# CoolMicApp/libcoolmic-dsp

Hardware: AMD Instinct MI355X
Metric: Msamples/s transform->vumeter (higher is better)
Workload: dtype int16

## Files before the change

### libcoolmic-dsp_amd/__init__.py

```python
import ctypes as C
import os

import numpy as np

_HERE = os.path.dirname(os.path.abspath(__file__))
LIB_PATH = os.environ.get("COOLMIC_HIP_LIB") or os.path.join(_HERE, "lib", "libcoolmic-dsp-hip.so")
if not os.path.exists(LIB_PATH):
    raise ImportError(
        f"{LIB_PATH} is missing: build it with `make -C {_HERE}` "
        "(or __graft_entry__.build()); there is no CPU fallback")

lib = C.CDLL(LIB_PATH)

MAX_CH = 16
ssize_t = C.c_ssize_t

ERROR_NONE, ERROR_GENERIC, ERROR_NOSYS, ERROR_FAULT = 0, -1, -8, -9
ERROR_INVAL, ERROR_NOMEM, ERROR_BUSY = -10, -11, -12

OUT_PCM, OUT_F32, VU, INPLACE, EQ, HOSTPCM, EXTSLOTS = 0x1, 0x2, 0x4, 0x8, 0x10, 0x20, 0x40
PLACE_SEARCH = 0x80
GEN_NULL, GEN_SINE, GEN_NOISE = 0, 1, 2
VU_FINISH_HOST, VU_FINISH_DEVICE = 0, 1
NODE_WORDS = 34
# ... 214 lines not shown
    "coolmic_group_get_iohandle": (_vp, [_vp, C.c_uint]),
    "coolmic_group_pump": (C.c_int, [_vp]),
    "coolmic_group_set_pull_threads": (C.c_int, [_vp, C.c_uint]),
    "coolmic_group_vumeter_result": (C.c_int, [_vp, C.c_uint, _P(VuResult)]),
    "coolmic_group_vumeter_results": (C.c_int, [_vp, _vp, _vp]),
    "coolmic_group_set_vu_finish": (C.c_int, [_vp, C.c_int]),
    "coolmic_group_set_true_peak": (C.c_int, [_vp, C.c_int]),
    "coolmic_group_true_peak": (C.c_int, [_vp, C.c_uint, _P(TruePeakResult)]),
    "coolmic_group_true_peaks": (C.c_int, [_vp, _vp, _vp]),
    "coolmic_group_set_loudness": (C.c_int, [_vp, C.c_int]),
    "coolmic_group_loudness": (C.c_int, [_vp, C.c_uint, _P(LoudnessResult)]),
    "coolmic_group_loudnesses": (C.c_int, [_vp, _vp, _vp]),
    "coolmic_group_loudness_set_weights": (C.c_int, [_vp, C.c_long, _vp]),
    "coolmic_group_loudness_reset": (C.c_int, [_vp, C.c_long]),
    "coolmic_group_streams": (C.c_uint, [_vp]),
}
MISSING = []
for _name, (_res, _args) in SIGNATURES.items():
    if not hasattr(lib, _name):
        MISSING.append(_name)
        continue
    _fn = getattr(lib, _name)
    _fn.restype = _res
    if _args is not None:
        _fn.argtypes = _args

if hasattr(lib, "cmhip_test_gain_consts"):
    lib.cmhip_test_gain_consts.restype = None
    lib.cmhip_test_gain_consts.argtypes = [C.c_uint16, C.c_uint16, _P(C.c_uint16), _P(C.c_uint32)]
if hasattr(lib, "cmhip_test_plan_run"):
    lib.cmhip_test_plan_run.restype = None
    lib.cmhip_test_plan_run.argtypes = [C.c_uint32, C.c_uint32, C.c_uint32, C.c_int, C.c_int, C.c_int, C.c_int,
                                        C.c_void_p]
lib.cmhip_test_merge_windows.restype = C.c_int
lib.cmhip_test_merge_windows.argtypes = [_P(C.c_uint64), C.c_uint, C.c_uint, C.c_uint, _P(VuResult)]
if hasattr(lib, "cmhip_test_unpack_finished"):
    lib.cmhip_test_unpack_finished.restype = C.c_int
    lib.cmhip_test_unpack_finished.argtypes = [_vp, C.c_uint, C.c_uint, C.c_uint, _vp, _vp]
    lib.cmhip_test_power_db_device.restype = C.c_int
    lib.cmhip_test_power_db_device.argtypes = [_vp, _vp, C.c_uint, _vp, _vp]
if hasattr(lib, "cmhip_test_plan_tpeak"):
    lib.cmhip_test_plan_tpeak.restype = None
    lib.cmhip_test_plan_tpeak.argtypes = [C.c_uint32, C.c_uint32, C.c_uint32, C.c_void_p]
    lib.cmhip_debug_tp_count.restype = C.c_ulonglong
    lib.cmhip_debug_tp_count.argtypes = []
if hasattr(lib, "cmhip_test_plan_loud"):
    lib.cmhip_test_plan_loud.restype = None
    lib.cmhip_test_plan_loud.argtypes = [C.c_uint32, C.c_uint32, C.c_uint32, C.c_void_p]
    lib.cmhip_debug_loud_count.restype = C.c_ulonglong
    lib.cmhip_debug_loud_count.argtypes = []
if hasattr(lib, "cmhip_test_plan_src"):
    lib.cmhip_test_plan_src.restype = None
    lib.cmhip_test_plan_src.argtypes = [C.c_uint32] * 6 + [C.c_void_p]
lib.cmhip_debug_run_count.restype = C.c_ulonglong
lib.cmhip_debug_run_count.argtypes = []
lib.coolmic_debug_vumeter_mode.restype = C.c_int
lib.coolmic_debug_vumeter_mode.argtypes = [_vp]
lib.coolmic_sine_period.restype = C.c_int
lib.coolmic_sine_period.argtypes = [C.c_uint32, _vp, _P(C.c_size_t)]


class CoolmicError(RuntimeError):
    def __init__(self, what, code):
        text = lib.coolmic_error2string(code).decode()
        detail = lib.cmhip_last_error().decode()
        super().__init__(f"{what}: {code} ({text}) {detail}")
# ... 2 lines not shown

def _check(what, rc):
    if rc != ERROR_NONE:
        raise CoolmicError(what, rc)


def device_count():
    return lib.cmhip_device_count()


def device_synchronize(device=0):
    _check("device_synchronize", lib.cmhip_device_synchronize(device))


def device_mem_info(device=0):
    f, t = C.c_size_t(), C.c_size_t()
    _check("device_mem_info", lib.cmhip_device_mem_info(device, C.byref(f), C.byref(t)))
    return f.value, t.value


def last_error():
    return lib.cmhip_last_error().decode()


def gain_consts(gain, scale):
    mi, mf = C.c_uint16(), C.c_uint32()
    lib.cmhip_test_gain_consts(gain, scale, C.byref(mi), C.byref(mf))
    return mi.value, mf.value


class RunPlan(C.Structure):
    _fields_ = [(name, C.c_int if name == "err" else C.c_uint32)
                for name in ("err", "family", "channels", "tile_u", "waves", "map", "stage", "grid", "block",
                             "chunks", "W", "rows_per_tile", "keep_flag")]


class TpPlan(C.Structure):
    _fields_ = [("err", C.c_int), ("fast", C.c_uint32), ("grid", C.c_uint32), ("block", C.c_uint32),
                ("chunks", C.c_uint32)]


def plan_tpeak(streams, channels, frames):
    p = TpPlan()
    lib.cmhip_test_plan_tpeak(streams, channels, frames, C.addressof(p))
    return p


def tp_dbtp(peak):
    return lib.cmhip_tp_dbtp(peak)


def tp_coefficients():
    h = np.zeros(48, dtype=np.int16)
    lib.cmhip_tp_coefficients(h.ctypes.data)
    return h.reshape(4, 12)


class LoudPlan(C.Structure):
    _fields_ = [("err", C.c_int), ("vec", C.c_uint32), ("grid", C.c_uint32), ("block", C.c_uint32)]


def plan_loud(streams, channels, frames):
    p = LoudPlan()
    lib.cmhip_test_plan_loud(streams, channels, frames, C.addressof(p))
    return p


# ... 17 lines not shown
class SrcPlan(C.Structure):
    _fields_ = [("err", C.c_int)] + [(n, C.c_uint32) for n in ("fast", "grid", "block", "chunks", "tile_out", "tile_in",
                                                               "row", "table_lds", "lds_bytes")]


def plan_src(streams, channels, L, M, T, out_frames):
    p = SrcPlan()
    lib.cmhip_test_plan_src(streams, channels, L, M, T, out_frames, C.addressof(p))
    return p


def src_design(rate_in, rate_out):
    L, M, T = C.c_uint(), C.c_uint(), C.c_uint()
    _check("src_design", lib.cmhip_src_design(rate_in, rate_out, C.byref(L), C.byref(M), C.byref(T), None, 0))
    h = np.zeros(L.value * T.value, dtype=np.int16)
    _check("src_design", lib.cmhip_src_design(rate_in, rate_out, None, None, None, h.ctypes.data, h.size))
    return L.value, M.value, T.value, h.reshape(L.value, T.value)


def src_out_frames(L, M, r, frames):
    return lib.cmhip_src_out_frames(L, M, r, frames)


RUN_FAMILIES = ("none", "fast", "fast_ro", "wide", "rows")


def plan_run(streams, channels, frames, out=False, f32=False, vu=False, identity_maps=True):
    p = RunPlan()
    lib.cmhip_test_plan_run(streams, channels, frames, int(bool(out)), int(bool(f32)), int(bool(vu)),
                            int(bool(identity_maps)), C.byref(p))
    d = {name: getattr(p, name) for name, _ in RunPlan._fields_}
    d["family"] = RUN_FAMILIES[d["family"]]
    return d


def merge_windows(windows, channels, rate=48000):
    import numpy as np
    w = np.ascontiguousarray(windows, dtype=np.uint64).reshape(-1, 33)
    r = VuResult()
    rc = lib.cmhip_test_merge_windows(w.ctypes.data_as(_P(C.c_uint64)), w.shape[0], channels, rate, C.byref(r))
    return rc, r


def unpack_finished(words, streams, channels, rate=48000, out=None):
    w = np.ascontiguousarray(words, dtype=np.uint64).reshape(-1)
    out = out if out is not None else (VuResult * streams)()
    rc = (C.c_int * streams)()
    _check("unpack_finished", lib.cmhip_test_unpack_finished(w.ctypes.data, streams, channels, rate, out, rc))
    return out, list(rc)


def power_db_device(sums, counts, want_log=False):
    s = np.ascontiguousarray(sums, dtype=np.uint64)
    c = np.ascontiguousarray(counts, dtype=np.uint64)
    assert s.shape == c.shape and s.ndim == 1
    db = np.empty(s.size, dtype=np.float64)
    lg = np.empty(s.size, dtype=np.float64) if want_log else None
    _check("power_db_device", lib.cmhip_test_power_db_device(s.ctypes.data, c.ctypes.data, s.size, db.ctypes.data,
                                                             lg.ctypes.data if want_log else None))
    return (db, lg) if want_log else db


def sine_period(rate):
    buf = np.zeros(96, dtype=np.int16)
    n = C.c_size_t()
    rc = lib.coolmic_sine_period(rate, buf.ctypes.data, C.byref(n))
# ... 728 lines not shown
```

### libcoolmic-dsp_amd/csrc/cmhip_device.h

```cpp
#ifndef CMHIP_DEVICE_H
#define CMHIP_DEVICE_H

#include "cmhip_internal.h"
#include <stdlib.h>
#include <type_traits>

namespace cmhip {

using u32 = uint32_t;
using u64 = unsigned long long;
typedef unsigned int u32x4 __attribute__((ext_vector_type(4)));
typedef unsigned int u32x2 __attribute__((ext_vector_type(2)));
typedef float f32x4 __attribute__((ext_vector_type(4)));


__device__ __forceinline__ u32 uniform(u32 v) { return __builtin_amdgcn_readfirstlane(v); }

__device__ __forceinline__ void done_epilogue(uint32_t *flag, uint32_t seq)
{
    if (flag) {
        __threadfence_system();
        __syncthreads();
        if (threadIdx.x == 0)
            __hip_atomic_store(flag, seq, __ATOMIC_RELEASE, __HIP_MEMORY_SCOPE_SYSTEM);
    }
}

__device__ __forceinline__ u64 make_key(u32 mag, u64 index, u32 neg)
{
    if (mag == 0)
        return 0;
    return ((u64)mag << KEY_ABS_SHIFT) | ((~index & KEY_IDX_MASK) << 1) | (u64)neg;
}


typedef short v2s __attribute__((ext_vector_type(2)));
typedef unsigned short v2u __attribute__((ext_vector_type(2)));

__device__ __forceinline__ u32 pk_sign(u32 w)
{
    v2s v = __builtin_bit_cast(v2s, w);
    v = v >> (short)15;
    return __builtin_bit_cast(u32, v);
}
__device__ __forceinline__ u32 pk_sub(u32 a, u32 b)
{
    v2u x = __builtin_bit_cast(v2u, a) - __builtin_bit_cast(v2u, b);
    return __builtin_bit_cast(u32, x);
}
// ... 59 lines not shown
__device__ __forceinline__ void with_gain_mode(u32 mode, F &&f)
{
    if constexpr (MODES) {
        if (mode == GAIN_IDENTITY)
            f(std::integral_constant<u32, GAIN_IDENTITY>{});
        else if (mode == GAIN_BELOW_SCALE)
            f(std::integral_constant<u32, GAIN_BELOW_SCALE>{});
        else
            f(std::integral_constant<u32, GAIN_GENERAL>{});
    } else {
        f(std::integral_constant<u32, GAIN_GENERAL>{});
    }
}

template <u32 N>
__device__ __forceinline__ int half_at(const u32 (&o)[N], u32 j)
{
    u32 w = 0;
#pragma unroll
    for (u32 i = 0; i < N; i++)
        if (i == (j >> 1))
            w = o[i];
    return (int)(short)(w >> (16u * (j & 1u)));
}

struct Extent {
    u32 nfr, nsamp;
    u32 nfull;
    u32 ntail;
};
__device__ __forceinline__ Extent stream_extent(const uint32_t *nframes, u32 frames, u32 s, u32 C)
{
    Extent e;
    e.nfr = nframes ? nframes[s] : frames;
    e.nsamp = e.nfr * C;
    e.nfull = e.nsamp >> 3;
    e.ntail = e.nsamp & 7u;
    return e;
}

__device__ __forceinline__ void load_vec(u32 (&x)[4], const int16_t *ins, u32 v, bool full, bool tail, u32 ntail)
{
    u32x4 w = {0, 0, 0, 0};
    if (full)
        w = __builtin_nontemporal_load(reinterpret_cast<const u32x4 *>(ins) + v);
    x[0] = w.x; x[1] = w.y; x[2] = w.z; x[3] = w.w;
    if (tail) {
        for (u32 j = 0; j < ntail; j++) {
            const u32 val = (u32)(uint16_t)ins[(u64)v * 8 + j];
#pragma unroll
            for (u32 i = 0; i < 4; i++)
                if (i == (j >> 1))
                    x[i] |= val << (16u * (j & 1u));
        }
    }
}
__device__ __forceinline__ void store_tail(int16_t *outs, u32 v, const u32 (&o)[4], u32 ntail)
{
    for (u32 j = 0; j < ntail; j++)
        outs[(u64)v * 8 + j] = (int16_t)half_at(o, j);
}

__device__ __forceinline__ u64 window_base(const RunArgs &a, VuState *vs, u32 k, u32 nsamp)
{
    const u64 base = vs->samples[a.parity];
    if (k == 0 && (threadIdx.x & 63u) == 0)
        vs->samples[a.parity ^ 1u] = base + nsamp;
    return base;
}

struct PeakAt {
    u32 u, lane, first, neg;
};
template <u32 NS, u32 TU>
__device__ __forceinline__ PeakAt locate_peak(u32 wkey, const u32 (&qw)[TU][4], const u32 (&x)[TU][4], u32 slot)
{
    const u32 mag = wkey >> 16;
    PeakAt p = {TU - 1u - ((wkey >> 6) & (TU - 1u)), 63u - (wkey & 63u), 8, 0};
    u32 Q[4], X[4];
#pragma unroll
    for (u32 u = 0; u < TU; u++) {
        if (p.u == u) {
#pragma unroll
            for (u32 i = 0; i < 4; i++) {
                Q[i] = (u32)__builtin_amdgcn_readlane((int)qw[u][i], (int)p.lane);
                X[i] = (u32)__builtin_amdgcn_readlane((int)x[u][i], (int)p.lane);
            }
        }
    }
#pragma unroll
    for (u32 j = 0; j < 8; j++) {
        if (j % NS != slot)
            continue;
        if (((u32)half_at(Q, j) & 0xffffu) == mag && p.first == 8) {
            p.first = j;
            p.neg = half_at(X, j) < 0 ? 1u : 0u;
        }
    }
    return p;
}

// ... 128 lines not shown
```

### libcoolmic-dsp_amd/csrc/cmhip_internal.h

```cpp
#pragma once

#include <hip/hip_runtime.h>
#include <hip/hip_ext.h>
#include <stdint.h>

namespace cmhip {

constexpr unsigned MAX_CH = 16;
constexpr unsigned MAX_EQ = 4;

struct alignas(128) StreamParam {
    uint32_t mode;
    uint32_t perm2;
    uint32_t map_identity;
    uint32_t mi01;
    uint32_t mf[MAX_CH];
    uint16_t mi[MAX_CH];
    uint8_t  chmap[MAX_CH];
};
static_assert(sizeof(StreamParam) == 128, "one line per stream");
constexpr uint32_t GAIN_GENERAL = 0, GAIN_BELOW_SCALE = 1, GAIN_IDENTITY = 2;

struct VuState {
    unsigned long long power[MAX_CH];
    unsigned long long key[MAX_CH];
    unsigned long long samples[2];
};

constexpr int      KEY_ABS_SHIFT = 47;
constexpr uint64_t KEY_IDX_MASK  = (1ull << 46) - 1;
constexpr int      NODE_KEY_ABS_SHIFT = 46;

struct EqParam {
    uint32_t nsec;
    float    coef[MAX_EQ][5];
};
struct EqState {
    float s[MAX_EQ][4];
};

struct RunArgs {
    const int16_t *in;
    int16_t       *out;
    float         *f32;
    const StreamParam *param;
    VuState       *vu;
    const uint32_t *nframes;
    uint32_t       frames;
    uint32_t       streams;
    uint32_t       channels;
    uint64_t       stride;
    uint64_t       plane;
    uint32_t       chunks;
    uint32_t       parity;
    uint32_t       identity_maps;
    uint32_t      *done_flag;
    uint32_t       done_seq;
};

struct EqArgs {
    const int16_t *in;
    int16_t       *out;
    float         *f32;
    const StreamParam *param;
    const EqParam *eq;
    EqState       *state;
    VuState       *vu;
    const uint32_t *nframes;
    uint32_t       frames;
    uint32_t       streams;
    uint32_t       channels;
    uint32_t       nsec;
    uint32_t       whole_streams;
    uint32_t       parity;
    uint64_t       stride;
    uint64_t       plane;
    uint32_t      *done_flag;
    uint32_t       done_seq;
};

constexpr unsigned TP_TAPS = 12;
constexpr unsigned TP_HIST = TP_TAPS - 1;
constexpr int16_t TP_P0[TP_TAPS] = {14, 90, -161, 272, -487, 1125, 7964, -838, 390, -218, 122, -68};
constexpr int16_t TP_P1[TP_TAPS] = {-239, 240, -424, 730, -1364, 3810, 6388, -1641, 832, -477, 271, -155};
constexpr int16_t tp_h(unsigned p, unsigned k)
{
    return p == 0 ? TP_P0[k] : p == 1 ? TP_P1[k] : p == 2 ? TP_P1[TP_TAPS - 1 - k] : TP_P0[TP_TAPS - 1 - k];
}

struct TpArgs {
// ... 47 lines not shown
    uint32_t       frames;
    uint32_t       streams;
    uint32_t       channels;
    uint32_t       parity;
    uint32_t       L, M, T;
    uint32_t       inv_l;
    uint32_t       chunks;
    uint32_t       tile_out;
    uint32_t       row;
    uint32_t       table_lds;
};

struct GenArgs {
    int16_t *dst;
    uint32_t streams, channels, frames;
    uint64_t stride;
    uint32_t seed;
    uint64_t first_global, global_step, frame_offset;
    int16_t  sine[48];
};

enum RunFamily : uint32_t { RUN_NONE = 0, RUN_FAST, RUN_FAST_RO, RUN_WIDE, RUN_ROWS };
struct RunPlan {
    hipError_t err;
    uint32_t   family;
    uint32_t   channels;
    uint32_t   tile_u;
    uint32_t   waves;
    uint32_t   map, stage;
    uint32_t   grid, block;
    uint32_t   chunks;
    uint32_t   W, rows_per_tile;
    uint32_t   keep_flag;
};
RunPlan plan_run(const RunArgs &a);
hipError_t launch_run(const RunArgs &a, hipStream_t st, hipEvent_t ev_start = nullptr, hipEvent_t ev_stop = nullptr,
                      bool *flagged = nullptr);
hipError_t prepare_eq(int device);
hipError_t launch_eq(const EqArgs &a, hipStream_t st, hipEvent_t ev_start = nullptr, hipEvent_t ev_stop = nullptr,
                     bool *flagged = nullptr);
struct TpPlan {
    hipError_t err;
    uint32_t   fast;
    uint32_t   grid, block;
    uint32_t   chunks;
};
TpPlan plan_tpeak(const TpArgs &a);
hipError_t launch_tpeak(const TpArgs &a, hipStream_t st);
struct LoudPlan {
    hipError_t err;
    uint32_t   vec;
    uint32_t   grid, block;
};
LoudPlan plan_loud(const LoudArgs &a);
hipError_t launch_loud(const LoudArgs &a, hipStream_t st);
struct SrcPlan {
    hipError_t err;
    uint32_t   fast;
    uint32_t   grid, block;
    uint32_t   chunks;
    uint32_t   tile_out;
    uint32_t   tile_in;
    uint32_t   row;
    uint32_t   table_lds;
    uint32_t   lds_bytes;
};
// ... 18 lines not shown
```

### libcoolmic-dsp_amd/csrc/k_block.hip

```cpp
#include "cmhip_device.h"

namespace cmhip {

constexpr u32 TILE_U_VUONLY = 16;

struct FastShare {
    u64 sum[2], key[2];
    u32 arrived;
};

template <int C, bool WRITE_PCM, bool WRITE_F32, bool DO_VU, int U, bool FULL>
__device__ __forceinline__ void fast_tile(const RunArgs &a, u32 s, u32 k, u32 nsamp, u32 nfull, u32 ntail,
                                          u64 base, VuState *vs, FastShare *share, const int16_t *a_in,
                                          int16_t *a_out, u64 a_stride)
{
    constexpr u32 TILE_U = U;
    constexpr u32 TILE_VEC = 64 * TILE_U;
    const u32 lane = threadIdx.x & 63u;
    const u32 v0 = k * TILE_VEC;

    const int16_t *ins = a_in + (u64)s * a_stride;
    int16_t *outs = WRITE_PCM ? a_out + (u64)s * a_stride : nullptr;
    u32x4 *dst = reinterpret_cast<u32x4 *>(outs);
    float *f32s = WRITE_F32 ? a.f32 + (u64)s * a.plane * C : nullptr;

    u32 x[TILE_U][4];
    bool full[TILE_U], tail[TILE_U];
#pragma unroll
    for (u32 u = 0; u < TILE_U; u++) {
        const u32 v = v0 + 64u * u + lane;
        full[u] = FULL || v < nfull;
        tail[u] = !FULL && ntail && v == nfull;
        load_vec(x[u], ins, v, full[u], tail[u], ntail);
    }

    __builtin_amdgcn_sched_barrier(0);
    (void)nsamp;
    const StreamParam *p = a.param + s;
    const u32 perm2 = p->perm2;
    constexpr bool ROLES = C == 2 && DO_VU && !WRITE_PCM && !WRITE_F32;
    const bool keep = ROLES && (perm2 == 0x03020100u || perm2 == 0x01000302u);
    const u32 sw = keep && perm2 == 0x01000302u ? 1u : 0u;
    const u32 mi01 = p->mi01;
    const u32 mf0 = p->mf[0], mf1 = p->mf[C - 1];
    const u32 mipk = C == 1 ? (mi01 & 0xffffu) * 0x10001u : (sw ? (mi01 >> 16) | (mi01 << 16) : mi01);
    const u32 mflo = sw ? mf1 : mf0, mfhi = sw ? mf0 : mf1;
    constexpr bool MODES = DO_VU && !WRITE_PCM && FULL;
    const u32 mode = MODES ? uniform(p->mode) : GAIN_GENERAL;

    if constexpr (ROLES) {
        if (!keep) {
#pragma unroll
            for (u32 u = 0; u < TILE_U; u++)
#pragma unroll
                for (u32 i = 0; i < 4; i++)
                    x[u][i] = __builtin_amdgcn_perm(x[u][i], x[u][i], perm2);
        }
    }

    u32 qw[TILE_U][4];
    PowAcc pw[2] = {{0, 0, 0}, {0, 0, 0}};
    u32 best[2] = {0, 0};
    __shared__ __attribute__((aligned(16))) float fst[WRITE_F32 && C == 1 && FULL ? 64 * 8 : 4];
    auto arithmetic = [&](auto mode_c) {
    constexpr u32 MODE = decltype(mode_c)::value;
#pragma unroll
    for (u32 u = 0; u < TILE_U; u++) {
        const u32 v = v0 + 64u * u + lane;
        u32 o[4], vmax = 0;
#pragma unroll
        for (u32 i = 0; i < 4; i++) {
// ... 44 lines not shown
            } else if constexpr (WRITE_F32) {
                store_f32<C>(f32s, a.plane, v, o);
            }
        } else if (tail[u]) {
            for (u32 j = 0; j < ntail; j++) {
                const int q = half_at(o, j);
                if constexpr (WRITE_PCM)
                    outs[(u64)v * 8 + j] = (int16_t)q;
                if constexpr (WRITE_F32)
                    f32s[(u64)(j % (u32)C) * a.plane + ((u64)v * 8 + j) / (u32)C] = q * (1.0f / 32768.0f);
            }
        }
    }
    };
    with_gain_mode<MODES>(mode, arithmetic);

    if constexpr (DO_VU) {
        pw[0].flush();
        pw[1].flush();
        u64 sum[2];
        u32 wkey[2];
        if constexpr (C == 1) {
            sum[0] = wave_add_u40(pw[0].total + pw[1].total);
            wkey[0] = wave_max_u32(max(best[0], best[1]));
            sum[1] = 0;
            wkey[1] = 0;
        } else {
            sum[0] = wave_add_u40(pw[0].total);
            sum[1] = wave_add_u40(pw[1].total);
            wkey[0] = wave_max_u32(best[0]);
            wkey[1] = wave_max_u32(best[1]);
        }
        u64 gkey[2] = {0, 0};
#pragma unroll
        for (int c = 0; c < C; c++) {
            const u32 mag = wkey[c] >> 16;
            if (mag == 0)
                continue;
            const PeakAt pk = locate_peak<(u32)C>(wkey[c], qw, x, (u32)c);
            gkey[c] = make_key(mag, base + 8ull * (v0 + 64u * pk.u + pk.lane) + (pk.first ^ sw), pk.neg);
        }
        if (lane < (u32)C) {
            const u64 ssum = (lane ^ sw) == 0 ? sum[0] : sum[1];
            const u64 skey = (lane ^ sw) == 0 ? gkey[0] : gkey[1];
            if (share) {
                if (ssum)
                    atomicAdd(&share->sum[lane], ssum);
                if (skey)
                    atomicMax(&share->key[lane], skey);
            } else {
                if (ssum)
                    atomicAdd(&vs->power[lane], ssum);
                if (skey)
                    atomicMax(&vs->key[lane], skey);
            }
        }
    }
}

template <int C, bool WRITE_PCM, bool WRITE_F32, bool DO_VU, int U, int NW = 1>
__device__ __forceinline__ void run_fast(const RunArgs &a)
{
    constexpr u32 TILE_VEC = 64 * U;
    static_assert(NW == 1 || !WRITE_F32, "the float-plane forms stage through LDS with one-wave barriers");
    const u32 lane = threadIdx.x & 63u;
    const int16_t *a_in = a.in;
    int16_t *a_out = a.out;
    const u64 a_stride = a.stride;
    const u32 a_frames = a.frames;
    u32 s, k;
    if constexpr (NW == 1) {
        s = blockIdx.x / a.chunks;
        k = blockIdx.x - s * a.chunks;
    } else {
        const u32 cw = (a.chunks + (u32)NW - 1u) / (u32)NW;
        s = blockIdx.x / cw;
        k = (blockIdx.x - s * cw) * (u32)NW + (threadIdx.x >> 6);
    }
    __shared__ FastShare shared_;
    FastShare *share = NW > 1 && DO_VU ? &shared_ : nullptr;
    if constexpr (NW > 1 && DO_VU) {
        if (threadIdx.x < 2u) {
            shared_.sum[threadIdx.x] = 0;
            shared_.key[threadIdx.x] = 0;
        }
        if (threadIdx.x == 0)
            shared_.arrived = 0;
        __syncthreads();
    }

    const Extent e = stream_extent(a.nframes, a_frames, s, (u32)C);
    const u32 nsamp = e.nsamp, nfull = e.nfull, ntail = e.ntail;
    const u32 v0 = k * TILE_VEC;

    VuState *vs = DO_VU ? a.vu + s : nullptr;
    u64 base = 0;
    if constexpr (DO_VU)
        base = window_base(a, vs, k, nsamp);
    if (v0 >= nfull + (ntail ? 1u : 0u)) {
        if constexpr (NW == 1)
            return;
    } else if (v0 + TILE_VEC <= nfull) {
        fast_tile<C, WRITE_PCM, WRITE_F32, DO_VU, U, true>(a, s, k, nsamp, nfull, ntail, base, vs, share, a_in, a_out, a_stride);
    } else {
        fast_tile<C, WRITE_PCM, WRITE_F32, DO_VU, U, false>(a, s, k, nsamp, nfull, ntail, base, vs, share, a_in, a_out, a_stride);
    }
    if constexpr (NW > 1 && DO_VU) {
        asm volatile("s_waitcnt lgkmcnt(0)" ::: "memory");
        u32 n = 0;
        if (lane == 0)
            n = atomicAdd(&shared_.arrived, 1u);
        n = (u32)__builtin_amdgcn_readfirstlane((int)n);
        asm volatile("" ::: "memory");
        if (n == (u32)NW - 1u && lane < (u32)C) {
            const u64 ssum = shared_.sum[lane], skey = shared_.key[lane];
            if (ssum)
                atomicAdd(&vs->power[lane], ssum);
            if (skey)
                atomicMax(&vs->key[lane], skey);
        }
    }
}

constexpr int FAST_WPE = 4;
template <int C, bool WRITE_PCM, bool WRITE_F32, bool DO_VU, int U, int NW = 1>
__global__ __launch_bounds__(64 * NW)
__attribute__((amdgpu_waves_per_eu(NW > 1 ? FAST_WPE : 1, NW > 1 ? FAST_WPE : 8))) void k_run_fast(RunArgs a)
{
    run_fast<C, WRITE_PCM, WRITE_F32, DO_VU, U, NW>(a);
    done_epilogue(a.done_flag, a.done_seq);
}
template <int C, int U>
__global__ __launch_bounds__(64) __attribute__((amdgpu_waves_per_eu(3))) void k_run_fast_ro(RunArgs a)
{
    run_fast<C, false, false, true, U>(a);
    done_epilogue(a.done_flag, a.done_seq);
}

constexpr u32 WIDE_TILE_U = 8;

template <int C, bool WRITE_PCM, bool WRITE_F32, bool DO_VU>
__global__ __launch_bounds__(64) void k_run_wide(RunArgs a)
{
    constexpr u32 TILE_U = WIDE_TILE_U;
    constexpr u32 TILE_VEC = 64 * TILE_U;
    constexpr u32 NS = C;
    constexpr u32 NG = NS / 2;
    const u32 lane = threadIdx.x;
    const u32 s = blockIdx.x / a.chunks;
    const u32 k = blockIdx.x - s * a.chunks;

    const Extent e = stream_extent(a.nframes, a.frames, s, (u32)C);
    const u32 nfull = e.nfull, ntail = e.ntail;
    const u32 v0 = k * TILE_VEC;

    VuState *vs = DO_VU ? a.vu + s : nullptr;
    u64 base = 0;
    if constexpr (DO_VU)
        base = window_base(a, vs, k, e.nsamp);
    if (v0 >= nfull + (ntail ? 1u : 0u)) {
        done_epilogue(a.done_flag, a.done_seq);
        return;
    }

    const StreamParam *p = a.param + s;
    u32 mipk[NG], mf[NS];
#pragma unroll
    for (u32 i = 0; i < NS; i++)
        mf[i] = p->mf[i];
#pragma unroll
    for (u32 g = 0; g < NG; g++)
        mipk[g] = (u32)p->mi[2u * g] | ((u32)p->mi[2u * g + 1u] << 16);

    const int16_t *ins = a.in + (u64)s * a.stride;
    int16_t *outs = WRITE_PCM ? a.out + (u64)s * a.stride : nullptr;
    u32x4 *dst = reinterpret_cast<u32x4 *>(outs);
    float *f32s = WRITE_F32 ? a.f32 + (u64)s * a.plane * C : nullptr;

    u32 x[TILE_U][4];
    bool full[TILE_U], tail[TILE_U];
#pragma unroll
    for (u32 u = 0; u < TILE_U; u++) {
        const u32 v = v0 + 64u * u + lane;
        full[u] = v < nfull;
        tail[u] = ntail && v == nfull;
        load_vec(x[u], ins, v, full[u], tail[u], ntail);
    }

    u32 qw[TILE_U][4];
    PowAcc pw[NS];
    u32 best[NS];
#pragma unroll
    for (u32 i = 0; i < NS; i++) {
        pw[i] = PowAcc{0, 0, 0};
        best[i] = 0;
    }
#pragma unroll
    for (u32 u = 0; u < TILE_U; u++) {
        const u32 v = v0 + 64u * u + lane;
        u32 o[4], vmax[NG];
#pragma unroll
        for (u32 g = 0; g < NG; g++)
            vmax[g] = 0;
#pragma unroll
        for (u32 i = 0; i < 4; i++) {
            constexpr u32 dummy = 0;
            (void)dummy;
            const u32 g = i % NG;
            qw[u][i] = gain2<true>(x[u][i], mipk[g], mf[2 * g], mf[2 * g + 1], o[i]);
            if constexpr (DO_VU) {
                vmax[g] = pk_max(vmax[g], qw[u][i]);
                pw[2 * g].add_lo(qw[u][i]);
                pw[2 * g + 1].add_hi(qw[u][i]);
            }
        }
        if constexpr (DO_VU) {
            const u32 tag = ((TILE_U - 1u - u) << 6) | (63u - lane);
#pragma unroll
            for (u32 g = 0; g < NG; g++) {
                best[2 * g] = max(best[2 * g], (vmax[g] << 16) | tag);
// ... 51 lines not shown
struct RowsVu {
    u64 pw[8];
    u32 best[8];
    u32 sv[4][4];
};

__device__ __forceinline__ void rows_vu_column(RowsVu &v, const u32 i, const u32 (&q)[4], const u32 (&o)[4],
                                               const u32 steptag)
{
    const u32 m = pk_max(pk_max(q[0], q[1]), pk_max(q[2], q[3]));
    const u32 klo = (m << 16) | steptag, khi = (m & 0xffff0000u) | steptag;
    const bool blo = klo > v.best[2 * i], bhi = khi > v.best[2 * i + 1];
    v.best[2 * i] = blo ? klo : v.best[2 * i];
    v.best[2 * i + 1] = bhi ? khi : v.best[2 * i + 1];
    const u32 mask = (blo ? 0xffffu : 0u) | (bhi ? 0xffff0000u : 0u);
#pragma unroll
    for (u32 u = 0; u < 4; u++)
        v.sv[i][u] = (o[u] & mask) | (v.sv[i][u] & ~mask);
    v.pw[2 * i] += sq_lo(q[2], sq_lo(q[1], sq_lo0(q[0])));
    v.pw[2 * i] += sq_lo0(q[3]);
    v.pw[2 * i + 1] += sq_hi(q[2], sq_hi(q[1], sq_hi0(q[0])));
    v.pw[2 * i + 1] += sq_hi0(q[3]);
}

template <bool WRITE_PCM, bool WRITE_F32, bool DO_VU, bool MAP, bool STAGE>
__global__ __launch_bounds__(64) void k_run_rows(RunArgs a, u32 W, u32 rows_per_tile)
{
    constexpr u32 UR = 4;
    __shared__ u64 lsum[MAX_CH];
    __shared__ u64 lkey[MAX_CH];
    __shared__ u32x4 raw[MAP ? UR * 64 : 1];
    __shared__ __attribute__((aligned(16))) float fstage[WRITE_F32 && STAGE ? UR * 8 * 64 : 4];
    const u32 lane = threadIdx.x;
    const u32 s = blockIdx.x / a.chunks;
    const u32 k = blockIdx.x - s * a.chunks;
    const u32 C = a.channels;

    const Extent e = stream_extent(a.nframes, a.frames, s, C);
    const u32 nfr = e.nfr, nfull = e.nfull, ntail = e.ntail;
    const u32 nvec = nfull + (ntail ? 1u : 0u);
    const u32 row0 = k * rows_per_tile;

    VuState *vs = DO_VU ? a.vu + s : nullptr;
    u64 base = 0;
    if constexpr (DO_VU)
        base = window_base(a, vs, k, e.nsamp);
    if ((u64)row0 * W >= nvec) {
        done_epilogue(a.done_flag, a.done_seq);
        return;
    }
    if constexpr (DO_VU) {
        if (lane < MAX_CH) {
            lsum[lane] = 0;
            lkey[lane] = 0;
        }
    }

    const StreamParam *p = a.param + s;
    const bool active = lane < W;
    const u32 lane_fr = 8u * lane / C;
    const u32 phase = 8u * lane - lane_fr * C;
    const u32 FW = 8u * W / C;
    constexpr bool MODES = DO_VU && !WRITE_PCM && !WRITE_F32;
    const u32 smode = uniform(p->mode);
    const u32 mode = MODES ? smode : GAIN_GENERAL;
    u32 ch[8], df[8], mipk[4], mf[8];
    u32 so[8];
#pragma unroll
    for (u32 j = 0; j < 8; j++) {
        const u32 t = phase + j;
        df[j] = t / C;
        ch[j] = t - df[j] * C;
        mf[j] = p->mf[ch[j]];
        so[j] = MAP ? 2u * ((lane_fr + df[j]) * C + p->chmap[ch[j]]) : 0u;
    }
    if (smode == GAIN_GENERAL) {
#pragma unroll
        for (u32 i = 0; i < 4; i++)
            mipk[i] = (u32)p->mi[ch[2 * i]] | ((u32)p->mi[ch[2 * i + 1]] << 16);
    } else {
#pragma unroll
        for (u32 i = 0; i < 4; i++)
            mipk[i] = smode == GAIN_IDENTITY ? 0x00010001u : 0u;
    }

    const int16_t *ins = a.in + (u64)s * a.stride;
    const u32x4 *src = reinterpret_cast<const u32x4 *>(ins);
    int16_t *outs = WRITE_PCM ? a.out + (u64)s * a.stride : nullptr;
    u32x4 *dst = reinterpret_cast<u32x4 *>(outs);
    float *f32s = WRITE_F32 ? a.f32 + (u64)s * a.plane * C : nullptr;

// ... 213 lines not shown
        p.family = RUN_WIDE;
        p.channels = a.channels;
        p.tile_u = WIDE_TILE_U;
        tiles = (nvec + 64ull * p.tile_u - 1) / (64ull * p.tile_u);
    } else {
        p.family = RUN_ROWS;
        p.map = a.identity_maps ? 0u : 1u;
        p.stage = f32 && a.channels != 16 ? 1u : 0u;
        u32 g = a.channels, e = 8;
        while (e) {
            const u32 t = g % e;
            g = e;
            e = t;
        }
        const u32 P = a.channels / g;
        p.W = 64u - 64u % P;
        const bool ro = !pcm && !f32;
        const u64 rows = (nvec + p.W - 1) / p.W;
        if (ro) {
            const u64 nt = (rows + 63) / 64;
            p.rows_per_tile = (u32)(((rows + nt - 1) / nt + 3u) & ~3ull);
        } else {
            p.rows_per_tile = P == 1 ? (a.channels == 16 ? 16u : 32u) : (a.identity_maps ? 8u : 16u);
        }
        tiles = (rows + p.rows_per_tile - 1) / p.rows_per_tile;
    }
    if (tiles * a.streams >= (1ull << 31)) {
        RunPlan refused{};
        refused.err = hipErrorInvalidValue;
        return refused;
    }
    p.chunks = (u32)tiles;
    p.waves = waves;
    p.grid = a.streams * ((p.chunks + waves - 1u) / waves);
    p.block = 64u * waves;
    p.keep_flag = a.done_flag && p.grid == 1u;
    return p;
}

constexpr u32 IO_PCM = 1, IO_F32 = 2, IO_VU = 4;
using RunKernel = void (*)(RunArgs);
using RowsKernel = void (*)(RunArgs, u32, u32);
template <int C>
constexpr RunKernel fast_kernels[8] = {
    nullptr,
    k_run_fast<C, true, false, false, TILE_U>,
    k_run_fast<C, false, true, false, TILE_U>,
    k_run_fast<C, true, true, false, TILE_U>,
    nullptr,
    k_run_fast<C, true, false, true, TILE_U>,
    k_run_fast<C, false, true, true, TILE_U>,
    k_run_fast<C, true, true, true, TILE_U>,
};
constexpr RunKernel wide_kernels[2][8] = {
    {nullptr, k_run_wide<4, true, false, false>, nullptr, nullptr,
     nullptr, k_run_wide<4, true, false, true>, nullptr, nullptr},
    {nullptr, k_run_wide<8, true, false, false>, k_run_wide<8, false, true, false>, k_run_wide<8, true, true, false>,
     nullptr, k_run_wide<8, true, false, true>, k_run_wide<8, false, true, true>, k_run_wide<8, true, true, true>},
};
template <bool MAP>
constexpr RowsKernel rows_kernels[2][8] = {
    {nullptr, k_run_rows<true, false, false, MAP, false>, k_run_rows<false, true, false, MAP, false>,
     k_run_rows<true, true, false, MAP, false>, k_run_rows<false, false, true, MAP, false>,
     k_run_rows<true, false, true, MAP, false>, k_run_rows<false, true, true, MAP, false>,
     k_run_rows<true, true, true, MAP, false>},
    {nullptr, nullptr, k_run_rows<false, true, false, MAP, true>, k_run_rows<true, true, false, MAP, true>,
     nullptr, nullptr, k_run_rows<false, true, true, MAP, true>, k_run_rows<true, true, true, MAP, true>},
};

hipError_t launch_run(const RunArgs &a, hipStream_t st, hipEvent_t ev_start, hipEvent_t ev_stop, bool *flagged)
{
    const RunPlan p = plan_run(a);
    if (flagged)
        *flagged = p.keep_flag != 0;
    if (p.family == RUN_NONE)
        return p.err;
    RunArgs b = a;
    b.chunks = p.chunks;
    if (!p.keep_flag)
        b.done_flag = nullptr;
    auto launch = [&](auto kernel, auto... extra) {
        hipExtLaunchKernelGGL(kernel, dim3(p.grid), dim3(p.block), 0, st, ev_start, ev_stop, 0, b, extra...);
    };
    const u32 io = (a.out ? IO_PCM : 0u) | (a.f32 ? IO_F32 : 0u) | (a.vu ? IO_VU : 0u);
    const bool mono = p.channels == 1;
    switch (p.family) {
    case RUN_FAST:
        if (p.waves == FAST_NW)
            launch(mono ? k_run_fast<1, true, false, true, TILE_U, FAST_NW> : k_run_fast<2, true, false, true, TILE_U, FAST_NW>);
        else
            launch((mono ? fast_kernels<1> : fast_kernels<2>)[io]);
        break;
    case RUN_FAST_RO:
        launch(mono ? k_run_fast_ro<1, TILE_U_VUONLY> : k_run_fast_ro<2, TILE_U_VUONLY>);
        break;
    case RUN_WIDE:
        launch(wide_kernels[p.channels == 8][io]);
        break;
    case RUN_ROWS:
        launch((p.map ? rows_kernels<true> : rows_kernels<false>)[p.stage][io], p.W, p.rows_per_tile);
        break;
    }
    return hipGetLastError();
}

extern "C" void cmhip_test_plan_run(uint32_t streams, uint32_t channels, uint32_t frames, int out, int f32, int vu,
                                    int identity_maps, RunPlan *plan)
{
    static uint32_t word;
    RunArgs a{};
    a.out = out ? reinterpret_cast<int16_t *>(&word) : nullptr;
    a.f32 = f32 ? reinterpret_cast<float *>(&word) : nullptr;
    a.vu = vu ? reinterpret_cast<VuState *>(&word) : nullptr;
    a.frames = frames;
    a.streams = streams;
    a.channels = channels;
    a.identity_maps = identity_maps ? 1u : 0u;
    a.done_flag = &word;
    if (plan)
        *plan = plan_run(a);
}

}
```

Baseline: 1.577 million.

## Replace per-block integer division with host-precomputed magic multiply and scalarize kernel prologue

Block-to-(stream, tile) index mapping now uses a multiply-shift reciprocal computed on the host instead of a runtime 32-bit divide in every kernel. Kernel arguments are forced into scalar registers, stream parameters and frame counts are read through the constant address space, and the VU window base/advance is split so the advance store happens after loads are issued. RunArgs fields are reordered so the hot ones sit together. The intent is to shorten the per-block prologue in small-tile kernels, at the cost of more inline-asm constraints and an exactness assumption in the magic divisor.

```diff
diff --git a/libcoolmic-dsp_amd/__init__.py b/libcoolmic-dsp_amd/__init__.py
--- a/libcoolmic-dsp_amd/__init__.py
+++ b/libcoolmic-dsp_amd/__init__.py
@@ -270,6 +270,9 @@
     lib.cmhip_test_plan_run.restype = None
     lib.cmhip_test_plan_run.argtypes = [C.c_uint32, C.c_uint32, C.c_uint32, C.c_int, C.c_int, C.c_int, C.c_int,
                                         C.c_void_p]
+if hasattr(lib, "cmhip_test_tile_index"):
+    lib.cmhip_test_tile_index.restype = None
+    lib.cmhip_test_tile_index.argtypes = [C.c_uint32, _vp, C.c_uint32, _vp, _vp, _P(C.c_uint32), _P(C.c_uint32)]
 lib.cmhip_test_merge_windows.restype = C.c_int
 lib.cmhip_test_merge_windows.argtypes = [_P(C.c_uint64), C.c_uint, C.c_uint, C.c_uint, _P(VuResult)]
 if hasattr(lib, "cmhip_test_unpack_finished"):
@@ -338,7 +341,7 @@
 class RunPlan(C.Structure):
     _fields_ = [(name, C.c_int if name == "err" else C.c_uint32)
                 for name in ("err", "family", "channels", "tile_u", "waves", "map", "stage", "grid", "block",
-                             "chunks", "W", "rows_per_tile", "keep_flag")]
+                             "chunks", "W", "rows_per_tile", "keep_flag", "tile_div", "tile_mul", "tile_shift")]
 
 
 class TpPlan(C.Structure):
@@ -422,6 +425,14 @@
     d = {name: getattr(p, name) for name, _ in RunPlan._fields_}
     d["family"] = RUN_FAMILIES[d["family"]]
     return d
+
+
+def tile_index(divisor, blocks):
+    b = np.ascontiguousarray(blocks, dtype=np.uint32)
+    q, r = np.zeros_like(b), np.zeros_like(b)
+    mul, shift = C.c_uint32(), C.c_uint32()
+    lib.cmhip_test_tile_index(divisor, b.ctypes.data, b.size, q.ctypes.data, r.ctypes.data, C.byref(mul), C.byref(shift))
+    return q, r, mul.value, shift.value
 
 
 def merge_windows(windows, channels, rate=48000):
diff --git a/libcoolmic-dsp_amd/csrc/cmhip_device.h b/libcoolmic-dsp_amd/csrc/cmhip_device.h
--- a/libcoolmic-dsp_amd/csrc/cmhip_device.h
+++ b/libcoolmic-dsp_amd/csrc/cmhip_device.h
@@ -15,6 +15,14 @@
 
 
 __device__ __forceinline__ u32 uniform(u32 v) { return __builtin_amdgcn_readfirstlane(v); }
+
+template <class T>
+using const_as = const __attribute__((address_space(4))) T;
+template <class T>
+__device__ __forceinline__ const_as<T> *as_const(const T *p)
+{
+    return (const_as<T> *)p;
+}
 
 __device__ __forceinline__ void done_epilogue(uint32_t *flag, uint32_t seq)
 {
@@ -140,7 +148,7 @@
 __device__ __forceinline__ Extent stream_extent(const uint32_t *nframes, u32 frames, u32 s, u32 C)
 {
     Extent e;
-    e.nfr = nframes ? nframes[s] : frames;
+    e.nfr = nframes ? as_const(nframes)[s] : frames;
     e.nsamp = e.nfr * C;
     e.nfull = e.nsamp >> 3;
     e.ntail = e.nsamp & 7u;
@@ -169,12 +177,31 @@
         outs[(u64)v * 8 + j] = (int16_t)half_at(o, j);
 }
 
-__device__ __forceinline__ u64 window_base(const RunArgs &a, VuState *vs, u32 k, u32 nsamp)
-{
-    const u64 base = vs->samples[a.parity];
+__device__ __forceinline__ u64 window_base(const VuState *vs, u32 parity)
+{
+    const unsigned long long *slot = &vs->samples[parity];
+    asm("" : "+v"(slot));
+    return __hip_atomic_load(slot, __ATOMIC_RELAXED, __HIP_MEMORY_SCOPE_AGENT);
+}
+__device__ __forceinline__ void window_advance(VuState *vs, u32 parity, u32 k, u64 base, u32 nsamp)
+{
     if (k == 0 && (threadIdx.x & 63u) == 0)
-        vs->samples[a.parity ^ 1u] = base + nsamp;
-    return base;
+        vs->samples[parity ^ 1u] = base + nsamp;
+}
+__device__ __forceinline__ u64 uniform64(u64 v)
+{
+    return (u64)uniform((u32)v) | ((u64)uniform((u32)(v >> 32)) << 32);
+}
+
+__device__ __forceinline__ void tile_args_in_sgprs(const RunArgs &a)
+{
+    asm volatile("" ::"s"(a.in), "s"(a.out), "s"(a.param), "s"(a.vu), "s"(a.nframes), "s"(a.stride), "s"(a.frames),
+                 "s"(a.parity), "s"(a.tile_div), "s"(a.tile_mul), "s"(a.tile_shift));
+}
+__device__ __forceinline__ void tile_index(const RunArgs &a, u32 &s, u32 &k)
+{
+    s = tile_quot(blockIdx.x, a.tile_mul, a.tile_shift);
+    k = blockIdx.x - s * a.tile_div;
 }
 
 struct PeakAt {
diff --git a/libcoolmic-dsp_amd/csrc/cmhip_internal.h b/libcoolmic-dsp_amd/csrc/cmhip_internal.h
--- a/libcoolmic-dsp_amd/csrc/cmhip_internal.h
+++ b/libcoolmic-dsp_amd/csrc/cmhip_internal.h
@@ -39,23 +39,42 @@
     float s[MAX_EQ][4];
 };
 
+struct TileDiv {
+    uint32_t div, mul, shift;
+};
+inline TileDiv tile_divisor(uint32_t d)
+{
+    uint32_t l = 0;
+    while ((1ull << l) < d)
+        l++;
+    const uint64_t p = 1ull << (31u + l);
+    return TileDiv{d, (uint32_t)((p + d - 1u) / d), 31u + l};
+}
+__host__ __device__ inline uint32_t tile_quot(uint32_t b, uint32_t mul, uint32_t shift)
+{
+    return (uint32_t)(((uint64_t)b * mul) >> shift);
+}
+
 struct RunArgs {
     const int16_t *in;
     int16_t       *out;
+    const StreamParam *param;
+    VuState       *vu;
+    const uint32_t *nframes;
+    uint64_t       stride;
+    uint32_t       frames;
+    uint32_t       parity;
+    uint32_t       tile_div;
+    uint32_t       tile_mul;
+    uint32_t       tile_shift;
+    uint32_t       chunks;
+    uint32_t       channels;
+    uint32_t       streams;
     float         *f32;
-    const StreamParam *param;
-    VuState       *vu;
-    const uint32_t *nframes;
-    uint32_t       frames;
-    uint32_t       streams;
-    uint32_t       channels;
-    uint64_t       stride;
     uint64_t       plane;
-    uint32_t       chunks;
-    uint32_t       parity;
     uint32_t       identity_maps;
+    uint32_t       done_seq;
     uint32_t      *done_flag;
-    uint32_t       done_seq;
 };
 
 struct EqArgs {
@@ -169,6 +188,7 @@
     uint32_t   chunks;
     uint32_t   W, rows_per_tile;
     uint32_t   keep_flag;
+    TileDiv    tiles;
 };
 RunPlan plan_run(const RunArgs &a);
 hipError_t launch_run(const RunArgs &a, hipStream_t st, hipEvent_t ev_start = nullptr, hipEvent_t ev_stop = nullptr,
diff --git a/libcoolmic-dsp_amd/csrc/k_block.hip b/libcoolmic-dsp_amd/csrc/k_block.hip
--- a/libcoolmic-dsp_amd/csrc/k_block.hip
+++ b/libcoolmic-dsp_amd/csrc/k_block.hip
@@ -8,19 +8,30 @@
     u64 sum[2], key[2];
     u32 arrived;
 };
+__device__ __forceinline__ void share_open(FastShare *share)
+{
+    if (threadIdx.x < 2u) {
+        share->sum[threadIdx.x] = 0;
+        share->key[threadIdx.x] = 0;
+    }
+    if (threadIdx.x == 0)
+        share->arrived = 0;
+    asm volatile("s_waitcnt lgkmcnt(0)" ::: "memory");
+    __builtin_amdgcn_s_barrier();
+    asm volatile("" ::: "memory");
+}
 
 template <int C, bool WRITE_PCM, bool WRITE_F32, bool DO_VU, int U, bool FULL>
 __device__ __forceinline__ void fast_tile(const RunArgs &a, u32 s, u32 k, u32 nsamp, u32 nfull, u32 ntail,
-                                          u64 base, VuState *vs, FastShare *share, const int16_t *a_in,
-                                          int16_t *a_out, u64 a_stride)
+                                          u64 vbase, VuState *vs, FastShare *share)
 {
     constexpr u32 TILE_U = U;
     constexpr u32 TILE_VEC = 64 * TILE_U;
     const u32 lane = threadIdx.x & 63u;
     const u32 v0 = k * TILE_VEC;
 
-    const int16_t *ins = a_in + (u64)s * a_stride;
-    int16_t *outs = WRITE_PCM ? a_out + (u64)s * a_stride : nullptr;
+    const int16_t *ins = a.in + (u64)s * a.stride;
+    int16_t *outs = WRITE_PCM ? a.out + (u64)s * a.stride : nullptr;
     u32x4 *dst = reinterpret_cast<u32x4 *>(outs);
     float *f32s = WRITE_F32 ? a.f32 + (u64)s * a.plane * C : nullptr;
 
@@ -35,8 +46,12 @@
     }
 
     __builtin_amdgcn_sched_barrier(0);
-    (void)nsamp;
-    const StreamParam *p = a.param + s;
+    if constexpr (DO_VU)
+        window_advance(vs, a.parity, k, vbase, nsamp);
+    if (share)
+        share_open(share);
+    __builtin_amdgcn_sched_barrier(0);
+    const const_as<StreamParam> *p = as_const(a.param + s);
     const u32 perm2 = p->perm2;
     constexpr bool ROLES = C == 2 && DO_VU && !WRITE_PCM && !WRITE_F32;
     const bool keep = ROLES && (perm2 == 0x03020100u || perm2 == 0x01000302u);
@@ -147,6 +162,7 @@
             wkey[1] = wave_max_u32(best[1]);
         }
         u64 gkey[2] = {0, 0};
+        const u64 base = uniform64(vbase);
 #pragma unroll
         for (int c = 0; c < C; c++) {
             const u32 mag = wkey[c] >> 16;
@@ -179,46 +195,33 @@
     constexpr u32 TILE_VEC = 64 * U;
     static_assert(NW == 1 || !WRITE_F32, "the float-plane forms stage through LDS with one-wave barriers");
     const u32 lane = threadIdx.x & 63u;
-    const int16_t *a_in = a.in;
-    int16_t *a_out = a.out;
-    const u64 a_stride = a.stride;
-    const u32 a_frames = a.frames;
+    tile_args_in_sgprs(a);
     u32 s, k;
-    if constexpr (NW == 1) {
-        s = blockIdx.x / a.chunks;
-        k = blockIdx.x - s * a.chunks;
-    } else {
-        const u32 cw = (a.chunks + (u32)NW - 1u) / (u32)NW;
-        s = blockIdx.x / cw;
-        k = (blockIdx.x - s * cw) * (u32)NW + (threadIdx.x >> 6);
-    }
+    tile_index(a, s, k);
+    if constexpr (NW > 1)
+        k = k * (u32)NW + uniform(threadIdx.x >> 6);
     __shared__ FastShare shared_;
     FastShare *share = NW > 1 && DO_VU ? &shared_ : nullptr;
-    if constexpr (NW > 1 && DO_VU) {
-        if (threadIdx.x < 2u) {
-            shared_.sum[threadIdx.x] = 0;
-            shared_.key[threadIdx.x] = 0;
-        }
-        if (threadIdx.x == 0)
-            shared_.arrived = 0;
-        __syncthreads();
-    }
-
-    const Extent e = stream_extent(a.nframes, a_frames, s, (u32)C);
+
+    const Extent e = stream_extent(a.nframes, a.frames, s, (u32)C);
     const u32 nsamp = e.nsamp, nfull = e.nfull, ntail = e.ntail;
     const u32 v0 = k * TILE_VEC;
 
     VuState *vs = DO_VU ? a.vu + s : nullptr;
     u64 base = 0;
     if constexpr (DO_VU)
-        base = window_base(a, vs, k, nsamp);
+        base = window_base(vs, a.parity);
     if (v0 >= nfull + (ntail ? 1u : 0u)) {
+        if constexpr (DO_VU)
+            window_advance(vs, a.parity, k, base, nsamp);
+        if (share)
+            share_open(share);
         if constexpr (NW == 1)
             return;
     } else if (v0 + TILE_VEC <= nfull) {
-        fast_tile<C, WRITE_PCM, WRITE_F32, DO_VU, U, true>(a, s, k, nsamp, nfull, ntail, base, vs, share, a_in, a_out, a_stride);
+        fast_tile<C, WRITE_PCM, WRITE_F32, DO_VU, U, true>(a, s, k, nsamp, nfull, ntail, base, vs, share);
     } else {
-        fast_tile<C, WRITE_PCM, WRITE_F32, DO_VU, U, false>(a, s, k, nsamp, nfull, ntail, base, vs, share, a_in, a_out, a_stride);
+        fast_tile<C, WRITE_PCM, WRITE_F32, DO_VU, U, false>(a, s, k, nsamp, nfull, ntail, base, vs, share);
     }
     if constexpr (NW > 1 && DO_VU) {
         asm volatile("s_waitcnt lgkmcnt(0)" ::: "memory");
@@ -262,8 +265,9 @@
     constexpr u32 NS = C;
     constexpr u32 NG = NS / 2;
     const u32 lane = threadIdx.x;
-    const u32 s = blockIdx.x / a.chunks;
-    const u32 k = blockIdx.x - s * a.chunks;
+    tile_args_in_sgprs(a);
+    u32 s, k;
+    tile_index(a, s, k);
 
     const Extent e = stream_extent(a.nframes, a.frames, s, (u32)C);
     const u32 nfull = e.nfull, ntail = e.ntail;
@@ -272,13 +276,15 @@
     VuState *vs = DO_VU ? a.vu + s : nullptr;
     u64 base = 0;
     if constexpr (DO_VU)
-        base = window_base(a, vs, k, e.nsamp);
+        base = window_base(vs, a.parity);
     if (v0 >= nfull + (ntail ? 1u : 0u)) {
+        if constexpr (DO_VU)
+            window_advance(vs, a.parity, k, base, e.nsamp);
         done_epilogue(a.done_flag, a.done_seq);
         return;
     }
 
-    const StreamParam *p = a.param + s;
+    const const_as<StreamParam> *p = as_const(a.param + s);
     u32 mipk[NG], mf[NS];
 #pragma unroll
     for (u32 i = 0; i < NS; i++)
@@ -301,6 +307,8 @@
         tail[u] = ntail && v == nfull;
         load_vec(x[u], ins, v, full[u], tail[u], ntail);
     }
+    if constexpr (DO_VU)
+        window_advance(vs, a.parity, k, base, e.nsamp);
 
     u32 qw[TILE_U][4];
     PowAcc pw[NS];
@@ -418,8 +426,9 @@
     __shared__ u32x4 raw[MAP ? UR * 64 : 1];
     __shared__ __attribute__((aligned(16))) float fstage[WRITE_F32 && STAGE ? UR * 8 * 64 : 4];
     const u32 lane = threadIdx.x;
-    const u32 s = blockIdx.x / a.chunks;
-    const u32 k = blockIdx.x - s * a.chunks;
+    tile_args_in_sgprs(a);
+    u32 s, k;
+    tile_index(a, s, k);
     const u32 C = a.channels;
 
     const Extent e = stream_extent(a.nframes, a.frames, s, C);
@@ -430,7 +439,9 @@
     VuState *vs = DO_VU ? a.vu + s : nullptr;
     u64 base = 0;
     if constexpr (DO_VU)
-        base = window_base(a, vs, k, e.nsamp);
+        base = window_base(vs, a.parity);
+    if constexpr (DO_VU)
+        window_advance(vs, a.parity, k, base, e.nsamp);
     if ((u64)row0 * W >= nvec) {
         done_epilogue(a.done_flag, a.done_seq);
         return;
@@ -442,7 +453,7 @@
         }
     }
 
-    const StreamParam *p = a.param + s;
+    const const_as<StreamParam> *p = as_const(a.param + s);
     const bool active = lane < W;
     const u32 lane_fr = 8u * lane / C;
     const u32 phase = 8u * lane - lane_fr * C;
@@ -722,7 +733,8 @@
     }
     p.chunks = (u32)tiles;
     p.waves = waves;
-    p.grid = a.streams * ((p.chunks + waves - 1u) / waves);
+    p.tiles = tile_divisor((p.chunks + waves - 1u) / waves);
+    p.grid = a.streams * p.tiles.div;
     p.block = 64u * waves;
     p.keep_flag = a.done_flag && p.grid == 1u;
     return p;
@@ -767,6 +779,9 @@
         return p.err;
     RunArgs b = a;
     b.chunks = p.chunks;
+    b.tile_div = p.tiles.div;
+    b.tile_mul = p.tiles.mul;
+    b.tile_shift = p.tiles.shift;
     if (!p.keep_flag)
         b.done_flag = nullptr;
     auto launch = [&](auto kernel, auto... extra) {
@@ -811,4 +826,18 @@
         *plan = plan_run(a);
 }
 
-}
+extern "C" void cmhip_test_tile_index(uint32_t divisor, const uint32_t *blocks, uint32_t n, uint32_t *quot, uint32_t *rem,
+                                      uint32_t *mul, uint32_t *shift)
+{
+    const TileDiv d = tile_divisor(divisor);
+    for (uint32_t i = 0; i < n; i++) {
+        quot[i] = tile_quot(blocks[i], d.mul, d.shift);
+        rem[i] = blocks[i] - quot[i] * d.div;
+    }
+    if (mul)
+        *mul = d.mul;
+    if (shift)
+        *shift = d.shift;
+}
+
+}
```

New measurement: 1.479 million. 0.937x the previous value.
